# lagodiuk/PipelineDP

Hardware: AMD Instinct MI355X
Metric: input rows/sec aggregated (whole node) + achieved HBM GB/s vs peak (higher is better)
Workload: dtype f64; 1 GPU; C3: DPEngine.aggregate COUNT+SUM+MEAN, Laplace, private partitions (truncated geometric), L0=2, Linf=1, 1e+09 rows in total, Zipf(1.1) partition keys; rows_per_gpu=1000000000, privacy_ids_per_gpu=10000000, partitions=1000000, parallelism=rows sharded by privacy_id over 1 GPU(s)

## Files before the change

pipelinedp_amd/csrc/pdp_bound.hip:

```cpp
#include <algorithm>
#include <cstdlib>
#include <type_traits>
#include <vector>

#include "pdp_internal.h"

namespace pdp {
namespace {

constexpr int kPartThreads = 512;
constexpr int kL1Threads = 1024;
constexpr int kL1Items = 8;
constexpr int kL1Rows = kL1Threads * kL1Items;
constexpr int kL2Items = 16;
constexpr int kL2Threads = 512;
constexpr int kL2Rows = kL2Threads * kL2Items;
constexpr int kL2GroupTiles = 16;
constexpr int kScanWaves = 16;
constexpr int kScanTiles = 16;
constexpr int kScanChunkTiles = kScanWaves * kScanTiles;
static_assert(kScanTiles % kL2GroupTiles == 0, "group starts must fall inside a wave's tiles");
constexpr int kTileRowBits = 16;
constexpr int64_t kTileRows = (int64_t)1 << kTileRowBits;
constexpr int kStagesPerTile = (int)(kTileRows / kL1Rows);
// ... 47 lines not shown
  static constexpr int kChunk = TH * kSieveChunkItems;
  static constexpr int kCap = TH * kSieveItems;
  static constexpr int kSlots = TH == 1024 ? 8 : 16;
  static constexpr int kSlotBits = TH == 1024 ? 3 : 4;
  static_assert((1 << kSlotBits) == kSlots, "slot bits");
  static_assert(kTileRows / kChunk <= kSlots || kTileRows / (kCap - kChunk + 1) + 1 <= kSlots,
                "sieve flushes per tile");
  static_assert(kCap <= 65535, "u16 run offsets");
};
constexpr int kSieveThreads2 = 512;
constexpr int64_t kSieveLds2 = 80 * 1024 - 256;
#ifndef PDP_L1_NT
#define PDP_L1_NT 1
#endif
#ifndef PDP_NT_BS
#define PDP_NT_BS 1
#endif

constexpr int64_t kSieveTileStride = kTileRows;
constexpr int64_t kBandTileStride = kTileRows;
constexpr int kSieveMaxT16 = 1 << 15;
constexpr int kBloomWords = 4096;
constexpr unsigned kBloomMaxIds = 8192;
constexpr int kRescanThreads = 512;
constexpr int kRescanBlocks = 1024;
constexpr int kSieveL2Groups = 4;
constexpr double kL2Target = 7000.0;
size_t sieve_stage_bytes(int key_format, int threads);
constexpr int kBandQueue = 128;
inline int64_t sieve_band_lds(int threads) { return (threads / 64) * kBandQueue * 8; }
inline int64_t sieve_lds(int key_format, int threads, int64_t n_buckets, bool u16, bool band) {
  return ((int64_t)sieve_stage_bytes(key_format, threads) + 7) / 8 * 8 + l1_hist_bytes(n_buckets, u16) +
         (band ? sieve_band_lds(threads) : 0);
}

struct Plan {
  int algorithm;
  int pk_bits;
  int bucket_bits;
  int super_bits;
  int rand_shift;
  int64_t n_buckets;
  int64_t n_supers;
  int64_t n_tiles;
  int64_t lds_bytes;
  int merge;
  int n_ranges;
  int range_bits;
  int two_level;
  int64_t n_fine;
  int64_t fine_items;
  int64_t range_group;
  int64_t n_groups;
  int key_format;
  int l1_local;
  int64_t n_stages;
  int sieve;
  int band;
  int64_t n_slots1;
  int64_t buckets_out;
  int l2_mult;
  int sieve_threads;
  int bucket_threads;
  int slot_bits;
  int hist_u16;
};

int64_t per_pid_lds(const pdp_bound_config* c) {
  const int64_t l0 = c->l0;
  const int64_t pair = 4 + (c->linf > 0 ? 8 * (int64_t)c->linf : 24);
  return l0 * 8 + l0 * pair;
}

bool test_hooks_enabled();
Plan make_plan(const pdp_bound_config* c) {
  Plan p{};
  p.pk_bits = bits_for(c->n_partitions);
  const int64_t per_pid = per_pid_lds(c);
  const int64_t n_ranges_est = (c->n_partitions + kRangeParts - 1) >> kRangeBits;
  p.bucket_threads = c->bucket_threads == kBucketThreads / 2 &&
                             (n_ranges_est <= kBucketThreads / 2 || n_ranges_est > kMaxRanges)
                         ? kBucketThreads / 2
                         : kBucketThreads;
  const int64_t max_pids = (p.bucket_threads == kBucketThreads ? kLdsBudget : kLdsBudget2) / per_pid;
  int s = -1, s2 = 0;
  if (max_pids >= 16) {
    s = 0;
    while (((int64_t)2 << s) <= max_pids) ++s;
    if (test_hooks_enabled()) {
      const char* e = std::getenv("PIPELINEDP_AMD_BUCKET_BITS");
      if (e != nullptr && std::atoi(e) >= 4 && std::atoi(e) < s) s = std::atoi(e);
    }
    const int u_bits = bits_for(c->n_privacy_ids);
    if (s > u_bits) s = u_bits;
    const int64_t nb = (c->n_privacy_ids + ((int64_t)1 << s) - 1) >> s;
    if (nb > kSingleLevelMax) {
      int lo = 1;
      while (((nb + ((int64_t)1 << lo) - 1) >> lo) > kMaxSupers) ++lo;
      double best = -1.0;
      for (int c = lo; c <= lo + 3 && ((int64_t)1 << c) < nb; ++c) {
        const double supers = (double)((nb + ((int64_t)1 << c) - 1) >> c);
        const double score = std::min((double)kL1Rows / supers, (double)kL2Rows / (double)((int64_t)1 << c));
        if (score > best) {
          best = score;
          s2 = c;
        }
// ... 72 lines not shown
  int t16 = 0;
  if (sieve_ok && c->sieve > 0) {
    t16 = c->sieve < kSieveMaxT16 ? c->sieve : kSieveMaxT16;
  } else if (sieve_ok && c->sieve == 0) {
    const double rows_per_id = (double)c->n_rows / (double)c->n_privacy_ids;
    const double want = c->l0 + 3.0 * std::sqrt((double)c->l0) + 3.0;
    const double t = want / (0.6 * rows_per_id);
    if (t <= 0.35) t16 = (int)std::ceil(t * 65536.0);
  }
  p.sieve = t16 > 0 ? t16 : 0;
  p.band = 0;
  if (p.sieve) {
    const int t2 = 2 * p.sieve < kSieveMaxT16 ? 2 * p.sieve : kSieveMaxT16;
    const bool fits = sieve_lds(p.key_format, kL1Threads, p.n_buckets, true, true) <= kL1LocalLds;
    const bool want = c->sieve_band > 0 || (c->sieve_band == 0 && p.sieve <= kSieveMaxT16 / 2);
    if (t2 > p.sieve && fits && want) p.band = t2;
  }
  p.sieve_threads = kL1Threads;
  p.hist_u16 = p.l1_local ? (int)l1_hist_u16(p.key_format, p.n_buckets) : 0;
  if (p.sieve) {
    const bool band = p.band != 0;
    p.hist_u16 = sieve_lds(p.key_format, kL1Threads, p.n_buckets, false, band) > kL1LocalLds;
    const bool u16_2 = sieve_lds(p.key_format, kSieveThreads2, p.n_buckets, false, band) > kSieveLds2;
    const bool fits2 = sieve_lds(p.key_format, kSieveThreads2, p.n_buckets, u16_2, band) <= kSieveLds2;
    if (fits2 && c->sieve_threads == kSieveThreads2) {
      p.sieve_threads = kSieveThreads2;
      p.hist_u16 = u16_2;
    }
  }
  p.slot_bits = p.sieve_threads == kSieveThreads2 ? SieveShape<kSieveThreads2>::kSlotBits
                                                   : SieveShape<kL1Threads>::kSlotBits;
  if (!p.sieve) p.slot_bits = 3;
  static_assert(kStagesPerTile == 8, "non-sieve level-1 stages per tile = 2^3");
  p.n_slots1 = p.sieve ? p.n_tiles << p.slot_bits : p.n_stages;
  p.buckets_out = p.sieve ? (p.band ? 3 : 2) * p.n_buckets : p.n_buckets;
  p.l2_mult = 1;
  if (p.sieve) {
    const double per_group = (double)kL2GroupTiles * (double)kTileRows * ((double)p.sieve / 65536.0) /
                             (double)(p.n_supers > 0 ? p.n_supers : 1);
    int m = (int)(kL2Target / (per_group > 1.0 ? per_group : 1.0));
    const int m_max = kL2Threads / (kL2GroupTiles << p.slot_bits);
    const int cap = kSieveL2Groups < m_max ? kSieveL2Groups : m_max;
    p.l2_mult = m < 1 ? 1 : (m > cap ? cap : m);
  }
  if (p.algorithm == PDP_ALGO_BUCKETED) {
    p.lds_bytes = ((p.lds_bytes + 7) & ~(int64_t)7) + (p.bucket_threads / 64) * kQueueCap * 12;
    p.lds_bytes += ((int64_t)8 << p.bucket_bits);
  }
  if (p.merge == PDP_MERGE_RANGES) {
    const int64_t recs = p.buckets_out * ((int64_t)c->l0 << p.bucket_bits);
    p.range_group = kRangeChunk;
    p.n_groups = recs / kRangeChunk + 2 * (int64_t)p.n_ranges + 1;
    p.fine_items = p.two_level ? recs / kRangeChunk + p.n_fine + 1 : 0;
  } else {
    p.n_ranges = 0;
    p.range_group = 0;
    p.n_groups = 0;
    p.two_level = 0;
    p.fine_items = 0;
  }
  return p;
}

struct Ws {
  uint64_t err;
  uint64_t sketch, cnt, rows, fsum, nsum, nsum2;
  uint64_t counts_tm, counts, chunk_sums, super_base, super_tm, super_off, keys1, rows1, keys2, rows2;
  uint64_t csum, gcur;
  uint64_t cand_key, cand_idx;
  uint64_t soff;
  uint64_t counts_tm2;
  uint64_t sbase, unres_bits, unres_list, sctl, fix_cnt, fix_cur;
  uint64_t fix_rec, fix_cap;
  uint64_t band, band_cnt, unres2_bits, unres2_list, sctl2, fix_cnt2, fix_cur2;
  uint64_t fix_blist;
  uint64_t tile_over;
  uint64_t runs, rec_key, rec_f0, rec_f1, rec_f2;
  uint64_t rr_items, rr_count;
  uint64_t fine_total, fine_chunks, fine_cur, stg_key, stg_f0, stg_f1, stg_f2, fine_items, fine_count;
  uint64_t item_hist;
  uint64_t total;
};

inline int64_t counts_stride(int64_t n_buckets) { return (n_buckets + 7) & ~(int64_t)7; }

Ws layout(const pdp_bound_config* c, const Plan& p) {
  Ws w{};
  uint64_t off = 0;
  w.err = off;
  off = align256(off + 16);
  if (p.algorithm == PDP_ALGO_GLOBAL_SKETCH) {
    const uint64_t slots = (uint64_t)c->n_privacy_ids * (uint64_t)c->l0;
    w.sketch = off; off = align256(off + slots * 8);
    w.cnt = off; off = align256(off + slots * 4);
    if (c->linf > 0) {
      w.rows = off; off = align256(off + slots * (uint64_t)c->linf * 8);
    } else {
      w.fsum = off; off = align256(off + slots * 8);
      w.nsum = off; off = align256(off + slots * 8);
      w.nsum2 = off; off = align256(off + slots * 8);
    }
  } else {
    const uint64_t n_counts = (uint64_t)counts_stride(p.n_buckets) * (uint64_t)p.n_tiles;
    const uint64_t n_chunks = ((uint64_t)p.n_buckets + kScanChunk - 1) / kScanChunk;
    const uint64_t n = (uint64_t)c->n_rows;
    w.counts_tm = off; off = align256(off + n_counts * 4);
    const bool u16 = p.hist_u16 != 0;
    if (p.l1_local && u16) { w.counts_tm2 = off; off = align256(off + n_counts * 4); }
    w.tile_over = off; off = align256(off + (uint64_t)p.n_tiles * 4);
    w.counts = off; off = align256(off + ((uint64_t)p.n_buckets + 1) * 4);
    w.chunk_sums = off; off = align256(off + (n_chunks + 1) * 4);
    const uint64_t n_sc = ((uint64_t)p.n_tiles + kScanChunkTiles - 1) / kScanChunkTiles;
    const uint64_t n_grp = ((uint64_t)p.n_tiles + kL2GroupTiles - 1) / kL2GroupTiles;
    w.csum = off; off = align256(off + n_sc * (uint64_t)p.n_buckets * 4);
    w.gcur = off; off = align256(off + n_grp * (uint64_t)p.n_buckets * 4);
    w.super_base = off; off = align256(off + (uint64_t)(p.n_supers + 1) * 4);
    w.super_tm = off; off = align256(off + (uint64_t)p.n_tiles * p.n_supers * 4);
    w.super_off = off; off = align256(off + (uint64_t)p.n_tiles * p.n_supers * 4);
    const bool packed = (p.key_format == PDP_KEYS_PACKED || p.key_format == PDP_KEYS_PACKED_WIDE ||
                         p.key_format == PDP_KEYS_PACKED64) && p.super_bits > 0;
    const uint64_t kb1 = p.key_format == PDP_KEYS_COMPACT ? 4 : 8;
    const uint64_t kb2 = (p.key_format == PDP_KEYS_WIDE || p.key_format == PDP_KEYS_PACKED_WIDE ||
                          p.key_format == PDP_KEYS_PACKED64) ? 8 : 4;
    const bool rows2 = p.key_format != PDP_KEYS_PACKED64;
    const uint64_t n1 = p.sieve ? (uint64_t)p.n_tiles * kSieveTileStride
                                : (p.l1_local ? (uint64_t)p.n_stages * kL1Rows : n);
    w.keys1 = off; off = align256(off + n1 * (packed ? 8 : kb1));
    if (!packed) { w.rows1 = off; off = align256(off + n1 * 4); }
    if (p.sieve) {
      if (off - w.keys1 < 8 * n) off = w.keys1 + align256(8 * n);
      w.fix_rec = w.keys1;
      w.fix_cap = (off - w.keys1) / 8;
    }
    if (p.l1_local) { w.soff = off; off = align256(off + (uint64_t)p.n_slots1 * (p.n_supers + 1) * 2); }
    if (p.sieve) {
      const uint64_t ids = (uint64_t)p.n_buckets << p.bucket_bits;
      w.sbase = off; off = align256(off + (uint64_t)p.n_slots1 * 4);
      w.unres_bits = off; off = align256(off + ids / 8);
      w.unres_list = off; off = align256(off + ids * 4);
      w.sctl = off; off = align256(off + 16);
      w.fix_cnt = off; off = align256(off + ((uint64_t)p.n_buckets + 1) * 4);
      w.fix_cur = off; off = align256(off + (uint64_t)p.n_buckets * 4);
      w.fix_blist = off; off = align256(off + ((uint64_t)p.n_buckets + 1) * 4);
      if (p.band) {
        w.band = off; off = align256(off + (uint64_t)p.n_tiles * kBandTileStride * 8);
        w.band_cnt = off; off = align256(off + (uint64_t)p.n_tiles * 4);
        w.unres2_bits = off; off = align256(off + ids / 8);
        w.unres2_list = off; off = align256(off + ids * 4);
        w.sctl2 = w.sctl + 8;
        w.fix_cnt2 = off; off = align256(off + ((uint64_t)p.n_buckets + 1) * 4);
        w.fix_cur2 = off; off = align256(off + (uint64_t)p.n_buckets * 4);
      }
    }
    if (p.super_bits > 0) {
      w.keys2 = off; off = align256(off + n * kb2);
      if (rows2) { w.rows2 = off; off = align256(off + n * 4); }
      else w.rows2 = w.keys2;
    } else {
      w.keys2 = w.keys1;
      w.rows2 = w.rows1;
    }
    w.cand_key = off; off = align256(off + n * kb2);
    w.cand_idx = off; off = align256(off + n * 4);
    if (p.merge == PDP_MERGE_RANGES) {
      const uint64_t recs = (uint64_t)p.buckets_out * ((uint64_t)c->l0 << p.bucket_bits);
      w.runs = off; off = align256(off + (uint64_t)p.buckets_out * (p.n_ranges + 1) * 4);
      w.rec_key = off; off = align256(off + recs * 8);
      if (c->flags & (PDP_ACC_SUM | PDP_SUM_PER_PARTITION)) { w.rec_f0 = off; off = align256(off + recs * 8); }
      if (c->flags & PDP_ACC_NSUM) { w.rec_f1 = off; off = align256(off + recs * 8); }
      if (c->flags & PDP_ACC_NSUM2) { w.rec_f2 = off; off = align256(off + recs * 8); }
      w.rr_items = off; off = align256(off + (uint64_t)p.n_groups * 16);
      w.rr_count = off; off = align256(off + 16);
      if (p.two_level) {
        const uint64_t nf = (uint64_t)p.n_fine;
        w.fine_total = off; off = align256(off + (nf + 1) * 4);
        w.fine_chunks = off; off = align256(off + (uint64_t)scan_chunk_sums_len((int64_t)nf) * 4);
        w.fine_cur = off; off = align256(off + nf * 4);
        w.stg_key = off; off = align256(off + recs * 8);
        if (w.rec_f0) { w.stg_f0 = off; off = align256(off + recs * 8); }
        if (w.rec_f1) { w.stg_f1 = off; off = align256(off + recs * 8); }
        if (w.rec_f2) { w.stg_f2 = off; off = align256(off + recs * 8); }
        w.fine_items = off; off = align256(off + (uint64_t)p.fine_items * 16);
        w.fine_count = off; off = align256(off + 16);
        const uint64_t F = (uint64_t)1 << (p.range_bits - kRangeBits);
        w.item_hist = off; off = align256(off + (uint64_t)p.n_groups * F * 4);
      }
    }
  }
  w.total = off;
  return w;
}

bool test_hooks_enabled() {
  const char* v = std::getenv("PIPELINEDP_AMD_TEST_HOOKS");
  return v != nullptr && v[0] == '1';
}

int validate(const pdp_bound_config* c) {
  if (c == nullptr) return set_error(PDP_E_INVALID, "config is NULL");
  if (c->n_rows < 0 || c->n_rows >= ((int64_t)1 << 32))
    return set_error(PDP_E_INVALID, "n_rows must be in [0, 2^32)");
  if (c->n_privacy_ids < 1 || c->n_privacy_ids >= ((int64_t)1 << 40))
    return set_error(PDP_E_INVALID, "n_privacy_ids must be in [1, 2^40)");
  if (c->n_partitions < 1 || c->n_partitions >= ((int64_t)1 << 32))
    return set_error(PDP_E_INVALID, "n_partitions must be in [1, 2^32)");
  if (c->l0 < 0 || c->l0 > PDP_MAX_L0)
    return set_error(PDP_E_UNSUPPORTED, "l0 out of supported range [0, PDP_MAX_L0]");
  if (c->linf < 0 || c->linf > PDP_MAX_LINF)
    return set_error(PDP_E_UNSUPPORTED, "linf out of supported range [0, PDP_MAX_LINF]");
  if (c->max_contributions < 0 || c->max_contributions > PDP_MAX_CONTRIBUTIONS)
    return set_error(PDP_E_UNSUPPORTED, "max_contributions out of supported range [0, PDP_MAX_CONTRIBUTIONS]");
  if (c->value_kind < PDP_VALUE_NONE || c->value_kind > PDP_VALUE_I64)
    return set_error(PDP_E_INVALID, "bad value_kind");
  if (c->value_kind != PDP_VALUE_I64 && (c->flags & PDP_SUM_INT))
    return set_error(PDP_E_INVALID, "PDP_SUM_INT requires int64 values");
  if (c->algorithm < PDP_ALGO_AUTO || c->algorithm > PDP_ALGO_PAIR_TABLE)
    return set_error(PDP_E_INVALID, "bad algorithm");
  if (c->merge < PDP_MERGE_AUTO || c->merge > PDP_MERGE_RANGES)
    return set_error(PDP_E_INVALID, "bad merge");
  if (c->key_format < PDP_KEYS_AUTO || c->key_format > PDP_KEYS_PACKED64)
    return set_error(PDP_E_INVALID, "bad key_format");
  if (c->sieve_threads != 0 && c->sieve_threads != kSieveThreads2 && c->sieve_threads != kL1Threads)
    return set_error(PDP_E_INVALID, "sieve_threads must be 0, 512 or 1024");
  if (c->bucket_threads != 0 && c->bucket_threads != kBucketThreads / 2 && c->bucket_threads != kBucketThreads)
    return set_error(PDP_E_INVALID, "bucket_threads must be 0, 512 or 1024");
// ... 2087 lines not shown
    const uint64_t u = e >> 32;
    const uint32_t r = (uint32_t)e;
    const int64_t k = pk[r];
    const bool dead = k < 0 || k >= kp.P || (allowed != nullptr && allowed[k] == 0);
    const uint64_t lpk = (u & lmask) << kp.pk_bits;
    const int64_t b = (int64_t)(u >> kp.bucket_bits);
    const unsigned pos = fix_start[b] + atomicAdd(fix_cur + b, 1u);
    if constexpr (REC == kRecCompact)
      keys[pos] = (uint32_t)(dead ? (0x80000000ull | lpk) : (lpk | (uint64_t)k));
    else if constexpr (REC == kRecWide)
      keys[pos] = dead ? ((1ull << 63) | lpk) : (lpk | (uint64_t)k);
    else
      keys[pos] = dead ? ~0ull : (((uint64_t)r << kp.row_shift) | lpk | (uint64_t)k);
    if constexpr (REC != kRecP64) rows[pos] = r;
  }
}

constexpr int kFixRunRows = 16;
__global__ void __launch_bounds__(kBlock) k_fix_buckets(KP kp, const unsigned* __restrict__ fix_start,
                                                        unsigned* __restrict__ runs, int64_t run_stride,
                                                        unsigned* __restrict__ blist,
                                                        const unsigned* __restrict__ prev,
                                                        unsigned* __restrict__ bits2,
                                                        unsigned* __restrict__ list2,
                                                        unsigned* __restrict__ sctl2) {
  const int64_t b = (int64_t)blockIdx.x * blockDim.x + threadIdx.x;
  if (b >= kp.n_buckets) return;
  const bool empty = fix_start[b + 1] == fix_start[b];
  if (runs != nullptr && empty)
    for (int r = blockIdx.y; r <= kp.n_ranges; r += gridDim.y) runs[(int64_t)r * run_stride + b] = 0;
  if (blockIdx.y != 0) return;
  if (!empty) {
    blist[1 + atomicAdd(blist, 1u)] = (unsigned)b;
    return;
  }
  if (prev == nullptr) return;
  const int64_t id0 = b << kp.bucket_bits;
  for (int64_t w = 0; w < ((int64_t)1 << kp.bucket_bits) / 64; ++w) {
    const int64_t i0 = id0 + 64 * w;
    const uint2 pw = reinterpret_cast<const uint2*>(prev)[i0 >> 6];
    unsigned long long m = (unsigned long long)pw.x | ((unsigned long long)pw.y << 32);
    if (i0 + 64 > kp.U) m &= kp.U > i0 ? (1ULL << (kp.U - i0)) - 1 : 0ULL;
    reinterpret_cast<uint2*>(bits2)[i0 >> 6] = make_uint2((unsigned)m, (unsigned)(m >> 32));
    if (m == 0) continue;
    unsigned at = atomicAdd(sctl2, (unsigned)__popcll(m));
    for (; m; m &= m - 1) list2[at++] = (unsigned)(i0 + __ffsll((long long)m) - 1);
  }
}

__global__ void __launch_bounds__(kRangeThreads) k_range_plan(KP kp, const unsigned* __restrict__ runs,
                                                              uint4* __restrict__ items,
                                                              unsigned* __restrict__ n_items,
                                                              const unsigned* __restrict__ last_ids,
                                                              int64_t last_buckets) {
  __shared__ unsigned wsum[kRangeThreads / 64 + 1];
  __shared__ unsigned s_base;
  const int r = blockIdx.x;
  const int64_t stride = kp.n_buckets;
  const int64_t n_buckets = last_ids != nullptr && *last_ids == 0u ? kp.n_buckets - last_buckets : kp.n_buckets;
  auto len_of = [&](int64_t b) -> unsigned {
    if (b >= n_buckets) return 0u;
    const unsigned* run = runs + r * stride + b;
    return run[stride] - run[0];
  };
  unsigned total = 0;
  for (int64_t c = 0; c < n_buckets; c += blockDim.x) {
    unsigned t;
    block_excl_scan(len_of(c + threadIdx.x), wsum, &t);
    total += t;
    __syncthreads();
  }
  if (total == 0) return;
  const unsigned C = (unsigned)kRangeChunk;
  const unsigned K = (total + C - 1) / C;
  if (threadIdx.x == 0) s_base = atomicAdd(n_items, K + 1);
  __syncthreads();
  const unsigned base = s_base;
  if (threadIdx.x == 0) items[base] = make_uint4((unsigned)r, 0u, 0u, 0u);
  if (threadIdx.x == 0 && total % C != 0)
    items[base + K] = make_uint4((unsigned)r | 0x80000000u, (unsigned)n_buckets, total, 0u);
  unsigned carry = 0;
  for (int64_t c = 0; c < n_buckets; c += blockDim.x) {
    const int64_t b = c + threadIdx.x;
    const unsigned len = len_of(b);
    unsigned t;
    const unsigned ex = carry + block_excl_scan(len, wsum, &t);
    if (len > 0) {
      const unsigned e = ex + len;
      for (unsigned k = ex / C + 1; k * C <= e; ++k)
        items[base + k] = make_uint4((unsigned)r | (k == K ? 0x80000000u : 0u), (unsigned)(b + 1), e, 0u);
    }
    carry += t;
    __syncthreads();
  }
}

__device__ __forceinline__ unsigned item_order(unsigned i, unsigned n) {
  return (unsigned)(((uint64_t)i * 2147483647ull) % (uint64_t)n);
}

__global__ void __launch_bounds__(kReduceThreads) k_range_reduce(KP kp, PairRecords rec, const uint4* __restrict__ items,
                                                               const unsigned* __restrict__ n_items,
                                                               pdp_partition_accumulators acc, unsigned* err) {
  extern __shared__ unsigned long long smem[];
  double* s0 = (double*)smem;
  double* s1 = s0 + kRangeParts;
  double* s2 = s1 + kRangeParts;
  unsigned long long* start = (unsigned long long*)(s2 + kRangeParts);
  unsigned* pc = (unsigned*)(start + kReduceThreads);
  unsigned* cn = pc + kRangeParts;
  unsigned* pre = cn + kRangeParts;
  unsigned* wsum = pre + kReduceThreads;
  const unsigned n_it = *n_items;
  if (blockIdx.x >= n_it) return;
  const unsigned iw = item_order(blockIdx.x, n_it);
  const uint4 it = items[iw];
  if (it.x >> 31) return;
  const uint4 nx = items[iw + 1];
  const int r = (int)it.x;
  const int64_t b_lo = it.y, b_hi = nx.y;
  const unsigned item_total = nx.z - it.z;
  if (item_total == 0) return;
  const int flags = kp.clip.flags;
  const bool f0 = flags & (PDP_ACC_SUM | PDP_SUM_PER_PARTITION), f1 = flags & PDP_ACC_NSUM,
             f2 = flags & PDP_ACC_NSUM2, sum_int = flags & PDP_SUM_INT;
  const int64_t p0 = (int64_t)r << kRangeBits;
  const int64_t n_slots = (int64_t)kp.l0 << kp.bucket_bits;
  const bool direct = item_total < kRangeDirect;
  if (!direct) {
    for (int t = threadIdx.x; t < kRangeParts; t += blockDim.x) {
      pc[t] = 0;
      cn[t] = 0;
      s0[t] = 0.0;
      s1[t] = 0.0;
      s2[t] = 0.0;
// ... 592 lines not shown
      kind == kRecCompact ? (ranges ? (const void*)k_bucket_bound<VK, KA, true, kRecCompact>
                                   : (const void*)k_bucket_bound<VK, KA, false, kRecCompact>)
      : kind == kRecWide  ? (ranges ? (const void*)k_bucket_bound<VK, KA, true, kRecWide>
                                   : (const void*)k_bucket_bound<VK, KA, false, kRecWide>)
                         : (ranges ? (const void*)k_bucket_bound<VK, KA, true, kRecP64>
                                   : (const void*)k_bucket_bound<VK, KA, false, kRecP64>);
  PDP_HIP_CHECK(hipFuncSetAttribute(kern, hipFuncAttributeMaxDynamicSharedMemorySize, (int)p.lds_bytes));
  void* cand_key = ws + w.cand_key;
  unsigned* cand_idx = (unsigned*)(ws + w.cand_idx);
  unsigned* unres_bits = mk.bits;
  unsigned* unres_list = mk.list;
  unsigned* sctl = mk.sctl;
  unsigned* err = (unsigned*)(ws + w.err);
  unsigned long long* fix_rec = mk.fix_rec;
  const unsigned* prev = mk.prev;
  void* args[] = {(void*)&kp,       (void*)&keys,       (void*)&rows,       (void*)&offsets,
                  (void*)&value,    (void*)&acc,        (void*)&rec,        (void*)&cand_key,
                  (void*)&cand_idx, (void*)&unres_bits, (void*)&unres_list, (void*)&sctl,
                  (void*)&err,      (void*)&fix_rec,    (void*)&prev,       (void*)&blist};
  const int64_t grid = blist != nullptr ? std::min<int64_t>(p.n_buckets, device_cus()) : p.n_buckets;
  PDP_PROF_BEGIN(name, st);
  PDP_HIP_CHECK(hipLaunchKernel(kern, dim3((unsigned)grid), dim3((unsigned)p.bucket_threads), args,
                                (size_t)p.lds_bytes, st));
  PDP_PROF_END(st);
  PDP_HIP_CHECK(hipGetLastError());
  return PDP_OK;
}

PairRecords pair_records(char* ws, const Ws& w, const Plan& p) {
  PairRecords rec{};
  if (w.runs) {
    rec.runs = (unsigned*)(ws + w.runs);
    rec.run_stride = p.buckets_out;
    rec.key = (unsigned long long*)(ws + w.rec_key);
    rec.f0 = w.rec_f0 ? (double*)(ws + w.rec_f0) : nullptr;
    rec.f1 = w.rec_f1 ? (double*)(ws + w.rec_f1) : nullptr;
    rec.f2 = w.rec_f2 ? (double*)(ws + w.rec_f2) : nullptr;
  }
  return rec;
}

template <int VK, bool KA>
int launch_buckets(const KP& kp, const Plan& p, hipStream_t st, const int64_t* pid, const int64_t* pk,
                   const uint8_t* allowed, const void* value, const pdp_partition_accumulators& acc, char* ws,
                   const Ws& w) {
  const PairRecords rec = pair_records(ws, w, p);
  unsigned long long* fix_rec = (unsigned long long*)(ws + w.fix_rec);
  Marks m1{w.unres_bits ? (unsigned*)(ws + w.unres_bits) : nullptr,
           w.unres_list ? (unsigned*)(ws + w.unres_list) : nullptr, w.sctl ? (unsigned*)(ws + w.sctl) : nullptr,
           nullptr, p.band ? fix_rec : nullptr};
  int rc = launch_bucket_kernel<VK, KA>(kp, p, st, ws + w.keys2, (const unsigned*)(ws + w.rows2),
                                        (const unsigned*)(ws + w.counts), value, acc, rec, ws, w, "k_bucket_bound", m1);
  if (rc != PDP_OK || !p.sieve) return rc;
  const int kind = rec_of(p.key_format);
  const int64_t n_slots = (int64_t)kp.l0 << kp.bucket_bits;
  auto fixup = [&](unsigned* bits, unsigned* sctl, unsigned* fix_cnt, unsigned* fix_cur, int seg, const Marks& mk,
                   int mark, const char* name) -> int {
    PDP_PROF_BEGIN("k_fix_filter", st);
    unsigned* blist = (unsigned*)(ws + w.fix_blist);
    hipLaunchKernelGGL(k_fix_filter, dim3(grid_for(kp.n, 1024)), dim3(kBlock), 0, st, kp, (const unsigned*)bits,
                       (const unsigned*)sctl, fix_rec, fix_cnt, (unsigned*)(ws + w.err), blist);
    PDP_PROF_END(st);
    PDP_HIP_CHECK(hipGetLastError());
    int r = scan_u32(fix_cnt, p.n_buckets, (unsigned*)(ws + w.chunk_sums), st);
    if (r != PDP_OK) return r;
    const unsigned fix_grid = grid_for(kp.n, 2048);
    PDP_PROF_BEGIN("k_fix_scatter", st);
    if (kind == kRecCompact)
      hipLaunchKernelGGL(k_fix_scatter<kRecCompact>, dim3(fix_grid), dim3(kBlock), 0, st, kp, pk, allowed,
                         (const unsigned long long*)fix_rec, (const unsigned*)sctl, (const unsigned*)fix_cnt, fix_cur,
                         (uint32_t*)(ws + w.keys2), (unsigned*)(ws + w.rows2));
    else if (kind == kRecWide)
      hipLaunchKernelGGL(k_fix_scatter<kRecWide>, dim3(fix_grid), dim3(kBlock), 0, st, kp, pk, allowed,
                         (const unsigned long long*)fix_rec, (const unsigned*)sctl, (const unsigned*)fix_cnt, fix_cur,
                         (unsigned long long*)(ws + w.keys2), (unsigned*)(ws + w.rows2));
    else
      hipLaunchKernelGGL(k_fix_scatter<kRecP64>, dim3(fix_grid), dim3(kBlock), 0, st, kp, pk, allowed,
                         (const unsigned long long*)fix_rec, (const unsigned*)sctl, (const unsigned*)fix_cnt, fix_cur,
                         (unsigned long long*)(ws + w.keys2), (unsigned*)(ws + w.rows2));
    PDP_PROF_END(st);
    PDP_HIP_CHECK(hipGetLastError());
    KP kf = kp;
    kf.sieve_mark = mark;
    kf.sieve_emit = 0;
    PairRecords fr = rec;
    fr.runs += seg * p.n_buckets;
    fr.key += seg * p.n_buckets * n_slots;
    if (fr.f0) fr.f0 += seg * p.n_buckets * n_slots;
    if (fr.f1) fr.f1 += seg * p.n_buckets * n_slots;
    if (fr.f2) fr.f2 += seg * p.n_buckets * n_slots;
    PDP_PROF_BEGIN("k_fix_buckets", st);
    hipLaunchKernelGGL(k_fix_buckets, dim3(grid_for(p.n_buckets), kFixRunRows), dim3(kBlock), 0, st, kf,
                       (const unsigned*)fix_cnt,
                       p.merge == PDP_MERGE_RANGES ? fr.runs : nullptr, fr.run_stride, blist,
                       mark ? mk.prev : nullptr, mk.bits, mk.list, mk.sctl);
    PDP_PROF_END(st);
    PDP_HIP_CHECK(hipGetLastError());
    Plan pf = p;
    if (p.merge != PDP_MERGE_RANGES || p.n_ranges <= kBucketThreads / 2) pf.bucket_threads = kBucketThreads / 2;
    return launch_bucket_kernel<VK, KA>(kf, pf, st, ws + w.keys2, (const unsigned*)(ws + w.rows2),
                                        (const unsigned*)fix_cnt, value, acc, fr, ws, w, name, mk, blist);
  };
  auto rescan = [&](const unsigned* bits, const unsigned* list, unsigned* sctl) {
    PDP_PROF_BEGIN("k_sieve_rescan", st);
    if (kp.keys_vec)
      hipLaunchKernelGGL(k_sieve_rescan<true>, dim3(kRescanBlocks), dim3(kRescanThreads), 0, st, kp, pid, bits, list,
                         sctl, fix_rec);
    else
      hipLaunchKernelGGL(k_sieve_rescan<false>, dim3(kRescanBlocks), dim3(kRescanThreads), 0, st, kp, pid, bits, list,
                         sctl, fix_rec);
    PDP_PROF_END(st);
  };
  unsigned* sctl = (unsigned*)(ws + w.sctl);
  unsigned* fix_cnt = (unsigned*)(ws + w.fix_cnt);
  unsigned* fix_cur = (unsigned*)(ws + w.fix_cur);
  const Marks none{m1.bits, m1.list, m1.sctl, nullptr, nullptr};
  if (!p.band) {
    rescan(m1.bits, m1.list, sctl);
    PDP_HIP_CHECK(hipGetLastError());
    return fixup(m1.bits, sctl, fix_cnt, fix_cur, 1, none, 0, "k_bucket_fix");
  }
  PDP_PROF_BEGIN("k_band_scan", st);
  hipLaunchKernelGGL(k_band_scan, dim3(kRescanBlocks), dim3(kRescanThreads), 0, st, kp,
                       (const unsigned long long*)(ws + w.band), (const unsigned*)(ws + w.band_cnt),
                       (const unsigned*)m1.bits, (const unsigned*)m1.list, sctl, fix_rec);
  PDP_PROF_END(st);
  PDP_HIP_CHECK(hipGetLastError());
  unsigned* sctl2 = (unsigned*)(ws + w.sctl2);
  const Marks m2{(unsigned*)(ws + w.unres2_bits), (unsigned*)(ws + w.unres2_list), sctl2, m1.bits, nullptr};
  rc = fixup(m1.bits, sctl, fix_cnt, fix_cur, 1, m2, 1, "k_bucket_fix");
  if (rc != PDP_OK) return rc;
  rescan(m2.bits, m2.list, sctl2);
  PDP_HIP_CHECK(hipGetLastError());
  return fixup(m2.bits, sctl2, (unsigned*)(ws + w.fix_cnt2), (unsigned*)(ws + w.fix_cur2), 2, m2, 0, "k_bucket_fix2");
}

int launch_merge(const KP& kp0, const Plan& p, hipStream_t st, char* ws, const Ws& w,
                 const pdp_partition_accumulators& acc) {
  KP kp = kp0;
  kp.n_buckets = p.buckets_out;
  const PairRecords rec = pair_records(ws, w, p);
  unsigned* err = (unsigned*)(ws + w.err);
  {
    PDP_HIP_CHECK(hipFuncSetAttribute((const void*)k_range_reduce, hipFuncAttributeMaxDynamicSharedMemorySize,
                                      (int)kRangeLds));
    uint4* items = (uint4*)(ws + w.rr_items);
    unsigned* n_items = (unsigned*)(ws + w.rr_count);
    PDP_HIP_CHECK(hipMemsetAsync(n_items, 0, 4, st));
    PDP_PROF_BEGIN("k_range_plan", st);
    const unsigned* last_ids = p.band ? (const unsigned*)(ws + w.sctl2) : nullptr;
    hipLaunchKernelGGL(k_range_plan, dim3((unsigned)p.n_ranges), dim3(kRangeThreads), 0, st, kp,
                       (const unsigned*)rec.runs, items, n_items, last_ids, (int64_t)p.n_buckets);
    PDP_PROF_END(st);
    PDP_HIP_CHECK(hipGetLastError());
    if (!p.two_level) {
      PDP_PROF_BEGIN("k_range_reduce", st);
      hipLaunchKernelGGL(k_range_reduce, dim3((unsigned)p.n_groups), dim3(kReduceThreads), kRangeLds, st, kp, rec,
                         (const uint4*)items, (const unsigned*)n_items, acc, err);
      PDP_PROF_END(st);
      PDP_HIP_CHECK(hipGetLastError());
      return PDP_OK;
    }
    unsigned* fine_total = (unsigned*)(ws + w.fine_total);
    unsigned* fine_cur = (unsigned*)(ws + w.fine_cur);
    PairRecords stg{};
    stg.key = (unsigned long long*)(ws + w.stg_key);
    stg.f0 = w.stg_f0 ? (double*)(ws + w.stg_f0) : nullptr;
    stg.f1 = w.stg_f1 ? (double*)(ws + w.stg_f1) : nullptr;
    stg.f2 = w.stg_f2 ? (double*)(ws + w.stg_f2) : nullptr;
    PDP_HIP_CHECK(hipMemsetAsync(fine_total, 0, (uint64_t)(p.n_fine + 1) * 4, st));
    PDP_PROF_BEGIN("k_split_count", st);
    unsigned* item_hist = (unsigned*)(ws + w.item_hist);
    hipLaunchKernelGGL(k_split_count, dim3((unsigned)p.n_groups), dim3(kSplitThreads), 0, st, kp, rec,
                       (const uint4*)items, (const unsigned*)n_items, fine_total, item_hist);
    PDP_PROF_END(st);
    PDP_HIP_CHECK(hipGetLastError());
    const int rc = scan_u32(fine_total, p.n_fine, (unsigned*)(ws + w.fine_chunks), st);
    if (rc != PDP_OK) return rc;
    PDP_HIP_CHECK(hipMemcpyAsync(fine_cur, fine_total, (uint64_t)p.n_fine * 4, hipMemcpyDeviceToDevice, st));
    PDP_PROF_BEGIN("k_split_scatter", st);
    if ((1 << (kp.range_bits - kRangeBits)) <= kSplitStageFan && PDP_SPLIT_STAGED)
      hipLaunchKernelGGL(k_split_scatter_staged, dim3((unsigned)p.n_groups), dim3(kSplitThreads), 0, st, kp, rec, stg,
                         (const uint4*)items, (const unsigned*)n_items, fine_cur, (const unsigned*)item_hist);
    else
      hipLaunchKernelGGL(k_split_scatter, dim3((unsigned)p.n_groups), dim3(kSplitThreads), 0, st, kp, rec, stg,
                         (const uint4*)items, (const unsigned*)n_items, fine_cur, (const unsigned*)item_hist);
    PDP_PROF_END(st);
    PDP_HIP_CHECK(hipGetLastError());
    uint4* fitems = (uint4*)(ws + w.fine_items);
    unsigned* n_fitems = (unsigned*)(ws + w.fine_count);
    PDP_HIP_CHECK(hipMemsetAsync(n_fitems, 0, 4, st));
    PDP_PROF_BEGIN("k_fine_plan", st);
    hipLaunchKernelGGL(k_fine_plan, dim3(grid_for(p.n_fine, 1 << 20)), dim3(kBlock), 0, st, kp,
                       (const unsigned*)fine_total, fitems, n_fitems);
    PDP_PROF_END(st);
    PDP_HIP_CHECK(hipGetLastError());
    PDP_HIP_CHECK(hipFuncSetAttribute((const void*)k_fine_reduce, hipFuncAttributeMaxDynamicSharedMemorySize,
                                      (int)kFineLds));
    PDP_PROF_BEGIN("k_fine_reduce", st);
    hipLaunchKernelGGL(k_fine_reduce, dim3((unsigned)p.fine_items), dim3(kReduceThreads), kFineLds, st, kp, stg,
                       (const uint4*)fitems, (const unsigned*)n_fitems, acc, err);
    PDP_PROF_END(st);
    PDP_HIP_CHECK(hipGetLastError());
  }
  return PDP_OK;
// ... 330 lines not shown
  if (rc != PDP_OK) return rc;
  if (info == nullptr) return set_error(PDP_E_INVALID, "info is NULL");
  if (pairs_mode(cfg)) {
    *info = pdp_bound_plan_info{};
    info->algorithm = PDP_ALGO_PAIR_TABLE;
    info->pk_bits = bits_for(cfg->n_partitions);
    return PDP_OK;
  }
  const Plan p = make_plan(cfg);
  info->algorithm = p.algorithm;
  info->bucket_bits = p.bucket_bits;
  info->rand_shift = p.rand_shift;
  info->pk_bits = p.pk_bits;
  info->n_buckets = p.algorithm == PDP_ALGO_BUCKETED ? p.n_buckets : 0;
  info->n_tiles = p.n_tiles;
  info->lds_bytes = p.algorithm == PDP_ALGO_BUCKETED ? p.lds_bytes : 0;
  info->merge = p.merge;
  info->n_ranges = p.n_ranges;
  info->range_group = p.range_group;
  info->key_format = p.key_format;
  info->sieve = p.sieve;
  info->band = p.band;
  info->sieve_threads = p.sieve ? p.sieve_threads : 0;
  info->bucket_threads = p.bucket_threads;
  info->hist_u16 = p.algorithm == PDP_ALGO_BUCKETED && p.l1_local ? p.hist_u16 : 0;
  info->reserved = 0;
  return PDP_OK;
}

int pdp_bound_workspace_bytes(const pdp_bound_config* cfg, uint64_t* bytes) {
  const int rc = validate(cfg);
  if (rc != PDP_OK) return rc;
  if (bytes == nullptr) return set_error(PDP_E_INVALID, "bytes is NULL");
  *bytes = pairs_mode(cfg) ? pairs_workspace_bytes(cfg) : layout(cfg, make_plan(cfg)).total;
  return PDP_OK;
}

int pdp_bound_contributions(const pdp_bound_config* cfg, const int64_t* privacy_id, const int64_t* partition_key,
                            const void* value, const uint8_t* pk_allowed, void* workspace,
                            uint64_t workspace_bytes, void* stream) {
  Plan p;
  Ws w;
  int rc = check_ws(cfg, workspace, workspace_bytes, &p, &w);
  if (rc != PDP_OK) return rc;
  if (cfg->n_rows > 0 && (partition_key == nullptr || (privacy_id == nullptr && !cfg->rows_are_units)))
    return set_error(PDP_E_INVALID, "key columns are NULL");
  if (cfg->value_kind != PDP_VALUE_NONE && cfg->n_rows > 0 && value == nullptr)
    return set_error(PDP_E_INVALID, "value column is NULL");
  if (cfg->value_kind == PDP_VALUE_NONE &&
      (cfg->flags & (PDP_ACC_SUM | PDP_ACC_NSUM | PDP_ACC_NSUM2 | PDP_SUM_PER_PARTITION)))
    return set_error(PDP_E_INVALID, "value sums requested without a value column");
  hipStream_t st = (hipStream_t)stream;
  char* ws = (char*)workspace;
  if (pairs_mode(cfg)) return pairs_bound(cfg, privacy_id, partition_key, value, pk_allowed, ws, st);
  KP kp = make_kp(cfg, p);
  kp.keys_vec = ((((uintptr_t)privacy_id) | ((uintptr_t)partition_key)) & 15) == 0;
  kp.fix_cap = (int64_t)w.fix_cap;
  if (test_hooks_enabled()) {
    const char* fc = std::getenv("PIPELINEDP_AMD_FIX_CAP");
    const long long v = fc != nullptr ? std::atoll(fc) : 0;
    if (v > 0 && v < kp.fix_cap) kp.fix_cap = v;
  }
  unsigned* err = (unsigned*)(ws + w.err);
  if (p.algorithm != PDP_ALGO_BUCKETED || cfg->n_rows == 0) PDP_HIP_CHECK(hipMemsetAsync(err, 0, 16, st));
  if (p.algorithm == PDP_ALGO_GLOBAL_SKETCH) {
    const uint64_t slots = (uint64_t)cfg->n_privacy_ids * (uint64_t)cfg->l0;
    PDP_HIP_CHECK(hipMemsetAsync(ws + w.sketch, 0xFF, slots * 8, st));
    PDP_HIP_CHECK(hipMemsetAsync(ws + w.cnt, 0, slots * 4, st));
    if (cfg->linf > 0) PDP_HIP_CHECK(hipMemsetAsync(ws + w.rows, 0xFF, slots * (uint64_t)cfg->linf * 8, st));
    else PDP_HIP_CHECK(hipMemsetAsync(ws + w.fsum, 0, w.total - w.fsum, st));
    if (cfg->n_rows == 0) return PDP_OK;
    PDP_PROF_BEGIN("k_pair_sketch", st);
    hipLaunchKernelGGL(k_pair_sketch, dim3(grid_for(cfg->n_rows)), dim3(kBlock), 0, st, kp, privacy_id,
                       partition_key, pk_allowed, (unsigned long long*)(ws + w.sketch), err);
    PDP_PROF_END(st);
    PDP_HIP_CHECK(hipGetLastError());
    return dispatch<GlobalRows>(cfg->value_kind, cfg->linf == 0, kp, st, privacy_id, partition_key, value,
                                pk_allowed, ws, w);
  }
  unsigned* counts = (unsigned*)(ws + w.counts);
  if (cfg->n_rows == 0) {
    PDP_HIP_CHECK(hipMemsetAsync(counts, 0, (p.n_buckets + 1) * 4, st));
    return PDP_OK;
  }
  {
    Fills f{};
    auto add = [&](uint64_t off, int64_t words, unsigned v) {
      f.p[f.k] = (unsigned*)(ws + off);
      f.n[f.k] = words;
      f.v[f.k] = v;
      ++f.k;
    };
    add(w.err, 4, 0u);
    if (p.l1_local) add(w.tile_over, p.n_tiles, ~0u);
    if (p.merge == PDP_MERGE_RANGES && p.sieve) {
      add(w.sctl, 4, 0u);
      add(w.fix_cnt, p.n_buckets + 1, 0u);
      add(w.fix_cur, p.n_buckets, 0u);
    }
    if (p.merge == PDP_MERGE_RANGES && p.band) {
      add(w.fix_cnt2, p.n_buckets + 1, 0u);
      add(w.fix_cur2, p.n_buckets, 0u);
    }
    const int rcf = launch_fills(f, st);
    if (rcf != PDP_OK) return rcf;
  }
// ... 115 lines not shown
```

pipelinedp_amd/csrc/pdp_internal.h:

```cpp
#pragma once

#include <hip/hip_runtime.h>
#include <stdint.h>

#include <cstdio>
#include <string>

#include "../../include/pipelinedp_amd.h"

namespace pdp {

int set_error(int code, const char* msg);

#define PDP_HIP_CHECK(expr)                                                        \
  do {                                                                             \
    hipError_t e_ = (expr);                                                        \
    if (e_ != hipSuccess) {                                                        \
      char buf_[256];                                                              \
      snprintf(buf_, sizeof(buf_), "%s failed: %s", #expr, hipGetErrorString(e_)); \
      return ::pdp::set_error(PDP_E_HIP, buf_);                                    \
    }                                                                              \
  } while (0)

constexpr uint64_t kEmpty = ~0ULL;
constexpr int kBlock = 256;

inline unsigned grid_for(int64_t n, int64_t cap = 1 << 16) {
  int64_t g = (n + kBlock - 1) / kBlock;
  if (g < 1) g = 1;
  if (g > cap) g = cap;
  return (unsigned)g;
}

inline uint64_t align256(uint64_t x) { return (x + 255) & ~(uint64_t)255; }

__device__ __forceinline__ longlong2 ld_nt(const longlong2* p) {
  typedef long long v2 __attribute__((ext_vector_type(2)));
  const v2 v = __builtin_nontemporal_load(reinterpret_cast<const v2*>(p));
  return make_longlong2(v.x, v.y);
}
__device__ __forceinline__ ulonglong2 ld_nt(const ulonglong2* p) {
  typedef unsigned long long v2 __attribute__((ext_vector_type(2)));
  const v2 v = __builtin_nontemporal_load(reinterpret_cast<const v2*>(p));
  return make_ulonglong2(v.x, v.y);
}
__device__ __forceinline__ uint4 ld_nt(const uint4* p) {
  typedef unsigned v4 __attribute__((ext_vector_type(4)));
  const v4 v = __builtin_nontemporal_load(reinterpret_cast<const v4*>(p));
  return make_uint4(v.x, v.y, v.z, v.w);
}
__device__ __forceinline__ uint2 ld_nt(const uint2* p) {
  typedef unsigned v2 __attribute__((ext_vector_type(2)));
  const v2 v = __builtin_nontemporal_load(reinterpret_cast<const v2*>(p));
  return make_uint2(v.x, v.y);
}
template <typename T>
__device__ __forceinline__ T ld_nt(const T* p) {
  return __builtin_nontemporal_load(p);
// ... 320 lines not shown
}

__device__ __forceinline__ PairSums pair_sums_from_totals(long long cnt, double fsum_or_bits, double nsum,
                                                          double nsum2, const ClipParams& cp) {
  PairSums s{cnt, 0, 0.0, nsum, nsum2};
  const long long ibits = __double_as_longlong(fsum_or_bits);
  if (cp.flags & PDP_SUM_PER_PARTITION) {
    if (cp.flags & PDP_SUM_INT) s.isum = clamp_ll(ibits, (long long)cp.min_sum, (long long)cp.max_sum);
    else s.fsum = fmin(fmax(fsum_or_bits, cp.min_sum), cp.max_sum);
  } else if (cp.flags & PDP_SUM_INT) {
    s.isum = ibits;
  } else {
    s.fsum = fsum_or_bits;
  }
  return s;
}

__device__ __forceinline__ void add_pair_to_partition(const pdp_partition_accumulators& acc, int64_t p,
                                                      const PairSums& s, int flags) {
  atomicAdd((unsigned long long*)(acc.privacy_id_count + p), 1ULL);
  if (acc.count) atomicAdd((unsigned long long*)(acc.count + p), (unsigned long long)s.count);
  if (acc.sum && (flags & (PDP_ACC_SUM | PDP_SUM_PER_PARTITION))) {
    if (flags & PDP_SUM_INT) atomicAdd((unsigned long long*)acc.sum + p, (unsigned long long)s.isum);
    else unsafeAtomicAdd((double*)acc.sum + p, s.fsum);
  }
  if (acc.normalized_sum && (flags & PDP_ACC_NSUM)) unsafeAtomicAdd(acc.normalized_sum + p, s.nsum);
  if (acc.normalized_sum_sq && (flags & PDP_ACC_NSUM2)) unsafeAtomicAdd(acc.normalized_sum_sq + p, s.nsum2);
}

int64_t scan_chunk_sums_len(int64_t n);
int scan_u32(unsigned* v, int64_t n, unsigned* chunk_sums, hipStream_t st);

#define PDP_SKETCH_MAX 256

inline bool pairs_mode(const pdp_bound_config* c) {
  return c->l0 == 0 || c->max_contributions > 0 || c->rows_are_units != 0 || c->l0 > PDP_SKETCH_MAX ||
         c->linf > PDP_SKETCH_MAX || c->algorithm == PDP_ALGO_PAIR_TABLE;
}
int pairs_validate(const pdp_bound_config* c);
uint64_t pairs_workspace_bytes(const pdp_bound_config* c);
int pairs_bound(const pdp_bound_config* c, const int64_t* pid, const int64_t* pk, const void* value,
                const uint8_t* allowed, char* ws, hipStream_t st);
int pairs_reduce(const pdp_bound_config* c, const void* value, char* ws, const pdp_partition_accumulators& acc,
                 hipStream_t st);

}

namespace pdp {
bool profiler_enabled();
void profiler_begin(const char* name, hipStream_t stream);
void profiler_end(hipStream_t stream);
}

#define PDP_PROF_BEGIN(name, stream) \
  do { if (::pdp::profiler_enabled()) ::pdp::profiler_begin(name, stream); } while (0)
#define PDP_PROF_END(stream) \
  do { if (::pdp::profiler_enabled()) ::pdp::profiler_end(stream); } while (0)
```

pipelinedp_amd/csrc/pdp_runtime.hip:

```cpp
#include <cstring>
#include <map>
#include <mutex>
#include <vector>

#include "pdp_internal.h"

namespace pdp {

namespace {
thread_local std::string g_last_error;
}

int set_error(int code, const char* msg) {
  g_last_error = msg;
  return code;
}

const char* last_error() { return g_last_error.c_str(); }

namespace {
struct ProfRecord {
  std::string name;
  hipEvent_t start, stop;
};
std::mutex g_prof_mu;
bool g_prof_on = false;
std::vector<ProfRecord> g_prof;
std::vector<hipEvent_t> g_free_events;
std::string g_open_name;
hipEvent_t g_open_start = nullptr;

hipEvent_t take_event() {
  if (!g_free_events.empty()) {
    hipEvent_t e = g_free_events.back();
    g_free_events.pop_back();
    return e;
  }
  hipEvent_t e = nullptr;
  if (hipEventCreate(&e) != hipSuccess) return nullptr;
  return e;
}
}

bool profiler_enabled() { return g_prof_on; }

void profiler_begin(const char* name, hipStream_t stream) {
  std::lock_guard<std::mutex> lock(g_prof_mu);
  g_open_start = take_event();
  g_open_name = name;
  if (g_open_start) (void)hipEventRecord(g_open_start, stream);
}

void profiler_end(hipStream_t stream) {
  std::lock_guard<std::mutex> lock(g_prof_mu);
  if (!g_open_start) return;
  hipEvent_t stop = take_event();
  if (!stop) return;
  (void)hipEventRecord(stop, stream);
  g_prof.push_back(ProfRecord{g_open_name, g_open_start, stop});
  g_open_start = nullptr;
}

namespace {
__device__ __forceinline__ int owner_of(int64_t z, int world) {
  z = (int64_t)((uint64_t)(z ^ (z >> 31)) * 0x9E3779B97F4A7C15ULL);
  z ^= z >> 29;
  int64_t r = z % world;
  return (int)(r < 0 ? r + world : r);
}

__global__ void __launch_bounds__(kBlock) k_owner_mismatches(const int64_t* __restrict__ ids, int64_t n, int world,
                                                             int rank, unsigned* out) {
  unsigned bad = 0;
  const int64_t stride = (int64_t)gridDim.x * blockDim.x;
  const bool vec = ((uintptr_t)ids & 15) == 0;
  const int64_t n2 = vec ? n / 2 : 0;
  for (int64_t i = blockIdx.x * (int64_t)blockDim.x + threadIdx.x; i < n2; i += stride) {
    const longlong2 v = reinterpret_cast<const longlong2*>(ids)[i];
    bad += (owner_of(v.x, world) != rank) + (owner_of(v.y, world) != rank);
  }
  for (int64_t i = 2 * n2 + blockIdx.x * (int64_t)blockDim.x + threadIdx.x; i < n; i += stride)
    bad += owner_of(ids[i], world) != rank;
  for (int off = 32; off > 0; off >>= 1) bad += __shfl_down(bad, off, 64);
  if ((threadIdx.x & 63) == 0 && bad) {
    unsigned old = __hip_atomic_load(out, __ATOMIC_RELAXED, __HIP_MEMORY_SCOPE_AGENT), assumed;
    do {
      assumed = old;
      const unsigned sum = assumed + bad < assumed ? 0xFFFFFFFFu : assumed + bad;
      old = atomicCAS(out, assumed, sum);
    } while (old != assumed);
  }
}
}

}

extern "C" {

int pdp_owner_mismatches(const int64_t* ids, int64_t n, int32_t world, int32_t rank, uint32_t* mismatches,
                         void* stream) {
  if (mismatches == nullptr || n < 0 || (n > 0 && ids == nullptr) || world < 1 || rank < 0 || rank >= world)
    return pdp::set_error(PDP_E_INVALID, "pdp_owner_mismatches: bad argument");
  hipStream_t st = (hipStream_t)stream;
  PDP_HIP_CHECK(hipMemsetAsync(mismatches, 0, 4, st));
  if (n == 0) return PDP_OK;
  const int64_t want = (n + 2 * pdp::kBlock - 1) / (2 * pdp::kBlock);
  const unsigned grid = (unsigned)(want < 4096 ? want : 4096);
  hipLaunchKernelGGL(pdp::k_owner_mismatches, dim3(grid), dim3(pdp::kBlock), 0, st, ids, n, (int)world, (int)rank,
                     mismatches);
  PDP_HIP_CHECK(hipGetLastError());
  return PDP_OK;
}

// ... 60 lines not shown
```

Baseline: 166.9 billion rows/s.

## Split range merge into two passes and overlap the first on a side stream

When the sieve and band paths are active without the two-level merge, the range merge is split into two passes. The first pass covers buckets up to n_buckets and the second covers the band buckets. The first pass runs on a side stream forked right after the bucket bound kernel, so it can overlap the sieve fixup work on the main stream. It then joins before returning. This hides merge latency behind fixup kernels, at the cost of an extra stream, events, a mutex, and duplicated plan/reduce launches over smaller groups.

```diff
diff --git a/pipelinedp_amd/csrc/pdp_bound.hip b/pipelinedp_amd/csrc/pdp_bound.hip
--- a/pipelinedp_amd/csrc/pdp_bound.hip
+++ b/pipelinedp_amd/csrc/pdp_bound.hip
@@ -123,6 +123,9 @@
   int64_t fine_items;
   int64_t range_group;
   int64_t n_groups;
+  int merge_split;
+  int64_t n_groups1;
+  int64_t n_groups2;
   int key_format;
   int l1_local;
   int64_t n_stages;
@@ -301,6 +304,12 @@
     p.range_group = kRangeChunk;
     p.n_groups = recs / kRangeChunk + 2 * (int64_t)p.n_ranges + 1;
     p.fine_items = p.two_level ? recs / kRangeChunk + p.n_fine + 1 : 0;
+    p.merge_split = p.sieve && p.band && !p.two_level;
+    if (p.merge_split) {
+      const int64_t per_bucket = (int64_t)c->l0 << p.bucket_bits;
+      p.n_groups1 = p.n_buckets * per_bucket / kRangeChunk + 2 * (int64_t)p.n_ranges + 1;
+      p.n_groups2 = (p.buckets_out - p.n_buckets) * per_bucket / kRangeChunk + 2 * (int64_t)p.n_ranges + 1;
+    }
   } else {
     p.n_ranges = 0;
     p.range_group = 0;
@@ -326,6 +335,7 @@
   uint64_t tile_over;
   uint64_t runs, rec_key, rec_f0, rec_f1, rec_f2;
   uint64_t rr_items, rr_count;
+  uint64_t rr_items2, rr_count2;
   uint64_t fine_total, fine_chunks, fine_cur, stg_key, stg_f0, stg_f1, stg_f2, fine_items, fine_count;
   uint64_t item_hist;
   uint64_t total;
@@ -420,6 +430,10 @@
       if (c->flags & PDP_ACC_NSUM2) { w.rec_f2 = off; off = align256(off + recs * 8); }
       w.rr_items = off; off = align256(off + (uint64_t)p.n_groups * 16);
       w.rr_count = off; off = align256(off + 16);
+      if (p.merge_split) {
+        w.rr_items2 = off; off = align256(off + (uint64_t)p.n_groups2 * 16);
+        w.rr_count2 = off; off = align256(off + 16);
+      }
       if (p.two_level) {
         const uint64_t nf = (uint64_t)p.n_fine;
         w.fine_total = off; off = align256(off + (nf + 1) * 4);
@@ -2613,19 +2627,19 @@
                                                               uint4* __restrict__ items,
                                                               unsigned* __restrict__ n_items,
                                                               const unsigned* __restrict__ last_ids,
-                                                              int64_t last_buckets) {
+                                                              int64_t last_buckets, int64_t b_first, int64_t b_end) {
   __shared__ unsigned wsum[kRangeThreads / 64 + 1];
   __shared__ unsigned s_base;
   const int r = blockIdx.x;
   const int64_t stride = kp.n_buckets;
-  const int64_t n_buckets = last_ids != nullptr && *last_ids == 0u ? kp.n_buckets - last_buckets : kp.n_buckets;
+  const int64_t n_buckets = last_ids != nullptr && *last_ids == 0u ? b_end - last_buckets : b_end;
   auto len_of = [&](int64_t b) -> unsigned {
     if (b >= n_buckets) return 0u;
     const unsigned* run = runs + r * stride + b;
     return run[stride] - run[0];
   };
   unsigned total = 0;
-  for (int64_t c = 0; c < n_buckets; c += blockDim.x) {
+  for (int64_t c = b_first; c < n_buckets; c += blockDim.x) {
     unsigned t;
     block_excl_scan(len_of(c + threadIdx.x), wsum, &t);
     total += t;
@@ -2637,11 +2651,11 @@
   if (threadIdx.x == 0) s_base = atomicAdd(n_items, K + 1);
   __syncthreads();
   const unsigned base = s_base;
-  if (threadIdx.x == 0) items[base] = make_uint4((unsigned)r, 0u, 0u, 0u);
+  if (threadIdx.x == 0) items[base] = make_uint4((unsigned)r, (unsigned)b_first, 0u, 0u);
   if (threadIdx.x == 0 && total % C != 0)
     items[base + K] = make_uint4((unsigned)r | 0x80000000u, (unsigned)n_buckets, total, 0u);
   unsigned carry = 0;
-  for (int64_t c = 0; c < n_buckets; c += blockDim.x) {
+  for (int64_t c = b_first; c < n_buckets; c += blockDim.x) {
     const int64_t b = c + threadIdx.x;
     const unsigned len = len_of(b);
     unsigned t;
@@ -3340,6 +3354,10 @@
   int rc = launch_bucket_kernel<VK, KA>(kp, p, st, ws + w.keys2, (const unsigned*)(ws + w.rows2),
                                         (const unsigned*)(ws + w.counts), value, acc, rec, ws, w, "k_bucket_bound", m1);
   if (rc != PDP_OK || !p.sieve) return rc;
+  if (p.merge_split && merge_overlap_enabled()) {
+    rc = merge_fork_record(ws, st);
+    if (rc != PDP_OK) return rc;
+  }
   const int kind = rec_of(p.key_format);
   const int64_t n_slots = (int64_t)kp.l0 << kp.bucket_bits;
   auto fixup = [&](unsigned* bits, unsigned* sctl, unsigned* fix_cnt, unsigned* fix_cur, int seg, const Marks& mk,
@@ -3429,6 +3447,49 @@
   kp.n_buckets = p.buckets_out;
   const PairRecords rec = pair_records(ws, w, p);
   unsigned* err = (unsigned*)(ws + w.err);
+  if (p.merge_split) {
+    PDP_HIP_CHECK(hipFuncSetAttribute((const void*)k_range_reduce, hipFuncAttributeMaxDynamicSharedMemorySize,
+                                      (int)kRangeLds));
+    auto pass = [&](int which, hipStream_t s) -> int {
+      uint4* items = (uint4*)(ws + (which == 0 ? w.rr_items : w.rr_items2));
+      unsigned* n_items = (unsigned*)(ws + (which == 0 ? w.rr_count : w.rr_count2));
+      const int64_t b_first = which == 0 ? 0 : p.n_buckets;
+      const int64_t b_end = which == 0 ? p.n_buckets : p.buckets_out;
+      const unsigned* last_ids = which == 1 && p.band ? (const unsigned*)(ws + w.sctl2) : nullptr;
+      PDP_HIP_CHECK(hipMemsetAsync(n_items, 0, 4, s));
+      PDP_PROF_BEGIN("k_range_plan", s);
+      hipLaunchKernelGGL(k_range_plan, dim3((unsigned)p.n_ranges), dim3(kRangeThreads), 0, s, kp,
+                         (const unsigned*)rec.runs, items, n_items, last_ids, (int64_t)p.n_buckets, b_first, b_end);
+      PDP_PROF_END(s);
+      PDP_HIP_CHECK(hipGetLastError());
+      PDP_PROF_BEGIN("k_range_reduce", s);
+      hipLaunchKernelGGL(k_range_reduce, dim3((unsigned)(which == 0 ? p.n_groups1 : p.n_groups2)),
+                         dim3(kReduceThreads), kRangeLds, s, kp, rec, (const uint4*)items, (const unsigned*)n_items,
+                         acc, err);
+      PDP_PROF_END(s);
+      PDP_HIP_CHECK(hipGetLastError());
+      return PDP_OK;
+    };
+    if (!merge_overlap_enabled()) {
+      const int rc = pass(0, st);
+      return rc != PDP_OK ? rc : pass(1, st);
+    }
+    std::lock_guard<std::mutex> lock(merge_side_mutex());
+    MergeSide* side = merge_side();
+    if (side == nullptr) return PDP_E_HIP;
+    if (side->fork_ws != ws || side->fork_st != st) PDP_HIP_CHECK(hipEventRecord(side->fork, st));
+    side->fork_ws = nullptr;
+    PDP_HIP_CHECK(hipStreamWaitEvent(side->stream, side->fork, 0));
+    int rc = pass(0, side->stream);
+    const hipError_t ej = hipEventRecord(side->join, side->stream);
+    if (rc == PDP_OK && ej == hipSuccess) rc = pass(1, st);
+    const hipError_t ew = ej == hipSuccess ? hipStreamWaitEvent(st, side->join, 0) : ej;
+    if (ew != hipSuccess) {
+      (void)hipStreamSynchronize(side->stream);
+      if (rc == PDP_OK) rc = set_error(PDP_E_HIP, "range merge: joining the side stream failed");
+    }
+    return rc;
+  }
   {
     PDP_HIP_CHECK(hipFuncSetAttribute((const void*)k_range_reduce, hipFuncAttributeMaxDynamicSharedMemorySize,
                                       (int)kRangeLds));
@@ -3438,7 +3499,8 @@
     PDP_PROF_BEGIN("k_range_plan", st);
     const unsigned* last_ids = p.band ? (const unsigned*)(ws + w.sctl2) : nullptr;
     hipLaunchKernelGGL(k_range_plan, dim3((unsigned)p.n_ranges), dim3(kRangeThreads), 0, st, kp,
-                       (const unsigned*)rec.runs, items, n_items, last_ids, (int64_t)p.n_buckets);
+                       (const unsigned*)rec.runs, items, n_items, last_ids, (int64_t)p.n_buckets, (int64_t)0,
+                       (int64_t)kp.n_buckets);
     PDP_PROF_END(st);
     PDP_HIP_CHECK(hipGetLastError());
     if (!p.two_level) {
@@ -3875,6 +3937,7 @@
     return set_error(PDP_E_INVALID, "value sums requested without a value column");
   hipStream_t st = (hipStream_t)stream;
   char* ws = (char*)workspace;
+  merge_fork_drop(ws);
   if (pairs_mode(cfg)) return pairs_bound(cfg, privacy_id, partition_key, value, pk_allowed, ws, st);
   KP kp = make_kp(cfg, p);
   kp.keys_vec = ((((uintptr_t)privacy_id) | ((uintptr_t)partition_key)) & 15) == 0;
diff --git a/pipelinedp_amd/csrc/pdp_internal.h b/pipelinedp_amd/csrc/pdp_internal.h
--- a/pipelinedp_amd/csrc/pdp_internal.h
+++ b/pipelinedp_amd/csrc/pdp_internal.h
@@ -4,6 +4,7 @@
 #include <stdint.h>
 
 #include <cstdio>
+#include <mutex>
 #include <string>
 
 #include "../../include/pipelinedp_amd.h"
@@ -430,6 +431,20 @@
 void profiler_end(hipStream_t stream);
 }
 
+namespace pdp {
+struct MergeSide {
+  hipStream_t stream = nullptr;
+  hipEvent_t fork = nullptr, join = nullptr;
+  const void* fork_ws = nullptr;
+  hipStream_t fork_st = nullptr;
+};
+bool merge_overlap_enabled();
+std::mutex& merge_side_mutex();
+MergeSide* merge_side();
+int merge_fork_record(const void* ws, hipStream_t st);
+void merge_fork_drop(const void* ws);
+}
+
 #define PDP_PROF_BEGIN(name, stream) \
   do { if (::pdp::profiler_enabled()) ::pdp::profiler_begin(name, stream); } while (0)
 #define PDP_PROF_END(stream) \
diff --git a/pipelinedp_amd/csrc/pdp_runtime.hip b/pipelinedp_amd/csrc/pdp_runtime.hip
--- a/pipelinedp_amd/csrc/pdp_runtime.hip
+++ b/pipelinedp_amd/csrc/pdp_runtime.hip
@@ -1,3 +1,4 @@
+#include <cstdlib>
 #include <cstring>
 #include <map>
 #include <mutex>
@@ -59,6 +60,59 @@
   (void)hipEventRecord(stop, stream);
   g_prof.push_back(ProfRecord{g_open_name, g_open_start, stop});
   g_open_start = nullptr;
+}
+
+namespace {
+std::mutex g_side_mu;
+std::map<int, MergeSide> g_sides;
+}
+
+bool merge_overlap_enabled() {
+  if (profiler_enabled()) return false;
+  const char* v = std::getenv("PIPELINEDP_AMD_MERGE_OVERLAP");
+  return !(v != nullptr && v[0] == '0');
+}
+
+std::mutex& merge_side_mutex() { return g_side_mu; }
+
+MergeSide* merge_side() {
+  int dev = 0;
+  if (hipGetDevice(&dev) != hipSuccess) {
+    set_error(PDP_E_HIP, "merge side stream: hipGetDevice failed");
+    return nullptr;
+  }
+  MergeSide& s = g_sides[dev];
+  if (s.stream == nullptr) {
+    MergeSide m;
+    if (hipStreamCreateWithFlags(&m.stream, hipStreamNonBlocking) != hipSuccess ||
+        hipEventCreateWithFlags(&m.fork, hipEventDisableTiming) != hipSuccess ||
+        hipEventCreateWithFlags(&m.join, hipEventDisableTiming) != hipSuccess) {
+      if (m.join) (void)hipEventDestroy(m.join);
+      if (m.fork) (void)hipEventDestroy(m.fork);
+      if (m.stream) (void)hipStreamDestroy(m.stream);
+      set_error(PDP_E_HIP, "merge side stream: cannot create the stream or its events");
+      return nullptr;
+    }
+    s = m;
+  }
+  return &s;
+}
+
+int merge_fork_record(const void* ws, hipStream_t st) {
+  std::lock_guard<std::mutex> lock(g_side_mu);
+  MergeSide* s = merge_side();
+  if (s == nullptr) return PDP_E_HIP;
+  s->fork_ws = nullptr;
+  PDP_HIP_CHECK(hipEventRecord(s->fork, st));
+  s->fork_ws = ws;
+  s->fork_st = st;
+  return PDP_OK;
+}
+
+void merge_fork_drop(const void* ws) {
+  std::lock_guard<std::mutex> lock(g_side_mu);
+  for (auto& kv : g_sides)
+    if (kv.second.fork_ws == ws) kv.second.fork_ws = nullptr;
 }
 
 namespace {
```

After: 168.8 billion rows/s (median of 6 runs). 1.01x the previous value.
